# hilo-mpc/hilo-mpc

Hardware: AMD Instinct MI355X
Metric: MPC steps/sec (batched instances, whole node) at fixed (nx,nu,N) (higher is better)
Workload: dtype f64

## Files before the change

hilo_mpc_amd/csrc/hilo_nmpc_track.h:

```cpp
#pragma once
#include "hilo_ocp.h"

namespace hilo {

template <class M, bool BIG_ = false, bool SYM_ = true>
struct NmpcTrack {
  using Model = M;
  static constexpr bool SYM = SYM_ && ModelSym<M>::value && !model_has_ext<M>::value;
  static constexpr int NX = M::NX, NU = M::NU, NZ = NX + NU, NPAR = M::NP + M::NU, NSD = 0;
  static constexpr bool FIX_X0 = true;
  static constexpr bool BIG = BIG_;
  static constexpr int NC = 0, NXV = NX, NX0 = NX, NU0 = NU;
  static constexpr bool COOP = model_has_ext<M>::value;
  static constexpr bool QUAD_COST = true;
  static constexpr int O_WZ = 0, O_ZREF = O_WZ + NZ * NZ, O_WN = O_ZREF + NZ, O_XREFN = O_WN + NX * NX,
                       O_WDU = O_XREFN + NX, O_HASDU = O_WDU + NU * NU, O_SZ = O_HASDU + 1, O_SDU = O_SZ + NZ * NZ;
  static constexpr bool SYMTAB = O_SDU + NU * NU <= OCP_NCOST;
  static constexpr int O_END = SYMTAB ? O_SDU + NU * NU : O_SZ;
  static constexpr int NCOST = O_END;

  template <class T, class E>
  __device__ __forceinline__ static void dyn(const OcpConst& pc, const double* par, const double*, int, const T* x,
                                             const T* u, T* xn, const E& ext) {
    T xp[NX], up[NU > 0 ? NU : 1], xo[NX];
#pragma unroll
    for (int i = 0; i < NX; ++i) xp[i] = x[i] * pc.sz[i];
#pragma unroll
    for (int i = 0; i < NU; ++i) up[i] = u[i] * pc.sz[NX + i];
    model_step<M>(pc.order, pc.nsub, xp, up, par, pc.dt, xo, ext);
#pragma unroll
    for (int i = 0; i < NX; ++i) xn[i] = xo[i] * rcp_fast(pc.sz[i]);
  }

  static constexpr bool PLANT = !COOP;
  __device__ __forceinline__ static void plant(const OcpConst& pc, const double* par, const double* x, const double* u, double* xn) {
    if constexpr (PLANT) {
      double xv[NX], uv[NU > 0 ? NU : 1], pv[M::NP > 0 ? M::NP : 1], xo[NX];
#pragma unroll
      for (int i = 0; i < NX; ++i) xv[i] = x[i];
#pragma unroll
      for (int i = 0; i < NU; ++i) uv[i] = u[i];
#pragma unroll
      for (int i = 0; i < M::NP; ++i) pv[i] = par[i];
      model_step<M>(pc.order, pc.nsub, xv, uv, pv, pc.dt, xo);
#pragma unroll
      for (int i = 0; i < NX; ++i) xn[i] = xo[i];
    }
  }

  template <class T>
  __device__ __forceinline__ static T stage_cost(const OcpConst& pc, const double* par, const double*, int k,
                                                 const T* x, const T* u) {
    T z[NZ];
#pragma unroll
// ... 10 lines not shown
        for (int j = 0; j < NZ; ++j) w[a][j] = pc.cost[O_WZ + (i0 + a < NZ ? i0 + a : i0) * NZ + j];
      asm volatile("");
#pragma unroll
      for (int a = 0; a < 2; ++a) {
        if (i0 + a < NZ) {
          T s = T(0.0);
#pragma unroll
          for (int j = 0; j < NZ; ++j) s = s + w[a][j] * z[j];
          acc = acc + z[i0 + a] * s;
        }
      }
    }
    if (k == 0 && pc.cost[O_HASDU] != 0.0) {
      T d[NU > 0 ? NU : 1];
#pragma unroll
      for (int i = 0; i < NU; ++i) d[i] = u[i] - par[M::NP + i];
#pragma unroll
      for (int i = 0; i < NU; ++i) {
        T s = T(0.0);
#pragma unroll
        for (int j = 0; j < NU; ++j) s = s + pc.cost[O_WDU + i * NU + j] * d[j];
        acc = acc + d[i] * s;
      }
    }
    return acc;
  }

  __device__ __forceinline__ static double cost_grad(const OcpConst& pc, const double* par, const double*, int k, int i, const double* z) {
    double g = 0.0;
    {
      double wr[NZ], wc[NZ], zr[NZ];
#pragma unroll
      for (int j = 0; j < NZ; ++j) { wr[j] = pc.cost[O_WZ + i * NZ + j]; wc[j] = pc.cost[O_WZ + j * NZ + i]; zr[j] = pc.cost[O_ZREF + j]; }
      asm volatile("");
#pragma unroll
      for (int j = 0; j < NZ; ++j) g += (wr[j] + wc[j]) * (z[j] - zr[j]);
    }
    if (k == 0 && i >= NX && pc.cost[O_HASDU] != 0.0) {
#pragma unroll
      for (int j = 0; j < NU; ++j)
        g += (pc.cost[O_WDU + (i - NX) * NU + j] + pc.cost[O_WDU + j * NU + (i - NX)]) * (z[NX + j] - par[M::NP + j]);
    }
    return g;
  }
  __device__ __forceinline__ static double cost_hess(const OcpConst& pc, int k, int i, int j) {
    double h = pc.cost[O_WZ + i * NZ + j] + pc.cost[O_WZ + j * NZ + i];
// ... 88 lines not shown
```

hilo_mpc_amd/csrc/hilo_ocp.h:

```cpp
#pragma once
#include "hilo_colloc.h"
#include "hilo_common.h"
#include "hilo_models.h"

namespace hilo {

constexpr int OCP_MAXNX = 12, OCP_MAXNU = 8, OCP_MAXNZ = OCP_MAXNX + OCP_MAXNU;
constexpr int OCP_FILTER = 16;
constexpr int OCP_MAXNC = 16;
#ifndef HILO_OCP_TPB
#define HILO_OCP_TPB 64
#endif
#ifndef HILO_OCP_MINW
#define HILO_OCP_MINW 1
#endif
#ifdef HILO_OCP_INLINE_PHASES
#define OCP_PHASE __attribute__((always_inline))
#else
#define OCP_PHASE __attribute__((noinline))
#endif
constexpr int OCP_TPB = HILO_OCP_TPB;
constexpr int OCP_NCOST = 2 * OCP_MAXNZ * OCP_MAXNZ + 4 * OCP_MAXNZ + 64;

struct OcpConst {
// ... 156 lines not shown
template <class PB, class = void> struct pb_nh { static constexpr int value = 0; };
template <class PB> struct pb_nh<PB, void_tt<decltype(PB::NH)>> { static constexpr int value = PB::NH; };
template <class PB, class = void> struct pb_sym { static constexpr bool value = false; };
template <class PB> struct pb_sym<PB, void_tt<decltype(PB::SYM)>> { static constexpr bool value = PB::SYM; };
template <class PB, class = void> struct pb_sym_mhe { static constexpr bool value = false; };
template <class PB> struct pb_sym_mhe<PB, void_tt<decltype(PB::SYM_MHE)>> { static constexpr bool value = PB::SYM_MHE; };
template <class PB, class = void> struct pb_vec_n { static constexpr int value = 0; };
template <class PB> struct pb_vec_n<PB, void_tt<decltype(PB::VEC_N)>> { static constexpr int value = PB::VEC_N; };
template <class PB, class = void> struct pb_fused_con { static constexpr bool value = false; };
template <class PB> struct pb_fused_con<PB, void_tt<decltype(PB::FUSED_CON)>> { static constexpr bool value = PB::FUSED_CON; };
template <class PB, class = void> struct pb_prep { static constexpr int value = 0; };
template <class PB> struct pb_prep<PB, void_tt<decltype(PB::PREP)>> { static constexpr int value = PB::PREP; };
template <class PB, class = void> struct pb_vec_max { static constexpr int value = 3; };
template <class PB> struct pb_vec_max<PB, void_tt<decltype(PB::VEC_MAX)>> { static constexpr int value = PB::VEC_MAX; };
template <class PB, class = void> struct pb_cstage { static constexpr int value = 0; };
template <class PB> struct pb_cstage<PB, void_tt<decltype(PB::CSTAGE)>> { static constexpr int value = PB::CSTAGE; };
template <class PB, class = void> struct pb_xcw { static constexpr int value = 0; };
template <class PB> struct pb_xcw<PB, void_tt<decltype(PB::XCW)>> { static constexpr int value = PB::XCW; };
template <class PB, class = void> struct pb_lam_fix { static constexpr bool value = false; };
template <class PB> struct pb_lam_fix<PB, void_tt<decltype(PB::LAM_FIX)>> { static constexpr bool value = PB::LAM_FIX; };
template <class PB, class = void> struct pb_fused { static constexpr bool value = false; };
template <class PB> struct pb_fused<PB, void_tt<decltype(PB::FUSED)>> { static constexpr bool value = PB::FUSED; };

__host__ __device__ constexpr size_t ocp_iter_doubles(int NX, int NU, int NC, int N) {
  const size_t NZ = NX + NU, NDIR = NZ * (NZ + 1) / 2, S = (size_t)(N + 1) * NZ;
  return 9 * S + NX + 5 * (size_t)N * NX + (size_t)N * NX * (NZ + 1) + (size_t)N * NZ * (NZ + 1) + (size_t)(N + 1) * NDIR +
         (size_t)(N + 1) * NX * (NX + 1) + (size_t)N * NU * (NX + 1) + (size_t)N * NX * (NX + 1) + (size_t)N * NC * (14 + NZ) +
         (size_t)N * 4 * NX;
}
__host__ __device__ constexpr size_t ocp_fixed_doubles(int NX, int NU, int NCONST, int NPAR, int NSD, int NEXT, int N, int NPREP = 0) {
  const size_t NZ = NX + NU;
  return NCONST + NZ * NZ + NZ + (N + 1) + 2 * 16 + 16 + NPAR + (size_t)(N + 1) * (NSD > 0 ? NSD : 0) + 1 + NEXT +
         (NZ * (NZ + 1) / 2 + 2) / 2 + NPREP;
}

struct OcpExtra {
  const double* par2;
  int npar1;
  int gather_stride;
  double* v_copy;
  double* gather;
  double* lam_x;
  double* g;
  const double* lbx;
  const double* ubx;
  long long bx_stride;
  double* x_next;
};

#ifdef HILO_OCP_DPROF
__device__ long long g_dprof[32];
#define DTICK(i) { if (blockIdx.x == 0 && threadIdx.x == 0) { const long long tn_ = clock64(); g_dprof[i] += tn_ - dt_; dt_ = tn_; } }
#define DTICK0 long long dt_ = clock64();
#define DTICKR dt_ = clock64();
#else
#define DTICK(i)
// ... 8 lines not shown
  static constexpr int NX = PB::NX, NU = PB::NU, NZ = NX + NU, NDIR = NZ * (NZ + 1) / 2, NXDIR = NX * (NX + 1) / 2;
  static constexpr int NPAR = PB::NPAR > 0 ? PB::NPAR : 1, NSD = PB::NSD;
  static constexpr bool FIX_X0 = PB::FIX_X0;
  static constexpr int NH = pb_nh<PB>::value;
  static constexpr bool FUSED = pb_fused<PB>::value;
  static constexpr bool FUSED_CON = pb_fused_con<PB>::value;
  static constexpr int PREP = pb_prep<PB>::value;
  static constexpr int XCW = pb_xcw<PB>::value;
#ifndef HILO_OCP_PREPB
#define HILO_OCP_PREPB 3
#endif
  static constexpr int PREPB = XCW > 0 ? HILO_OCP_PREPB : 1;
  static constexpr int PREPL = PREP * PREPB > pb_cstage<PB>::value ? PREP * PREPB : pb_cstage<PB>::value;
  static constexpr bool SYM = pb_sym<PB>::value;
  static constexpr bool SYM_MHE = pb_sym_mhe<PB>::value;
  static constexpr bool COOP = PB::COOP;
  static constexpr int NEXT_SCR = COOP ? 12 * OCP_TPB : 0;
  static constexpr int NEXT = COOP ? NEXT_SCR + GP2_HDR + 3 * GP2_MAXN : 0;
  static constexpr int NC = PB::NC;
  static_assert(NC <= OCP_MAXNC, "too many constraint rows");
  static constexpr int NXV = PB::NXV, NX0 = PB::NX0, NU0 = PB::NU0;
  static_assert(!COOP || (OCP_TPB == 64 && NDIR <= 64), "cooperative models need one wave per instance");
  static constexpr bool MFMA_STAGE = OCP_TPB == 64 && NZ + 1 <= 16 && NX <= 16;
  static constexpr int NCONST = (int)((__builtin_offsetof(OcpConst, cost) + sizeof(double) * PB::NCOST + 7) / 8);
  static constexpr int ABP = NZ + 1, WP = NZ + 1, PP = NX + 1;

  static constexpr bool BIG = PB::BIG;
  using dp = cond_t<BIG, gbl_double*, lds_double*>;
  using cdp = cond_t<BIG, gbl_cdouble*, lds_cdouble*>;
  static constexpr int VEC_N = pb_vec_n<PB>::value;
  __host__ __device__ static constexpr size_t vec_doubles_level(int N, int level) {
    return (level >= 1 ? 7 * (size_t)(N + 1) * NZ : 0) + (level >= 2 ? 3 * (size_t)N * NX : 0) + (level >= 3 ? (size_t)(N + 1) * NZ : 0);
  }
  static constexpr size_t VEC_BUDGET = 40 * 1024 - 64;
  static constexpr bool vec_fits(int level) {
    return (ocp_fixed_doubles(NX, NU, NCONST, NPAR, NSD, NEXT, VEC_N, PREPL) + vec_doubles_level(VEC_N, level)) * sizeof(double) <= VEC_BUDGET;
  }
  static constexpr int VEC_FIT = !(BIG && VEC_N > 0) ? 0 : (vec_fits(3) ? 3 : (vec_fits(2) ? 2 : (vec_fits(1) ? 1 : 0)));
  static constexpr int VEC_LEVEL = VEC_FIT < pb_vec_max<PB>::value ? VEC_FIT : pb_vec_max<PB>::value;
  static constexpr bool VEC_LDS = VEC_LEVEL > 0;
  __host__ __device__ static constexpr size_t vec_doubles(int N) { return vec_doubles_level(N, VEC_LEVEL); }
  using vp = cond_t<BIG && VEC_LEVEL < 1, gbl_double*, lds_double*>;
  using cvp = cond_t<BIG && VEC_LEVEL < 1, gbl_cdouble*, lds_cdouble*>;
  using ep = cond_t<BIG && VEC_LEVEL < 2, gbl_double*, lds_double*>;
  using gp_t = cond_t<BIG && VEC_LEVEL < 3, gbl_double*, lds_double*>;
  struct Lds {
    const __attribute__((address_space(3))) OcpConst* pc;
    vp Z, Zt, D, zL, zU;
    vp lbA, ubA;
    ep lam, c, ct;
    gp_t grad;
    dp lamn, AB, W, Qd, P, Kg, sig, rbN, Acl;
    dp Xs;
    dp prep;
    dp xc;
    lds_double* prepl;
    lds_double* gpc;
    dp cs, cst, cnu, cnun, cvL, cvU, cdvL, cdvU, cds, cd, csig, crb, Jd;
    dp c0, cd0, cdt;
    lds_double *Mm, *mm, *fk, *filt, *red, *par, *sd, *ext;
    __attribute__((address_space(3))) int* dirs;
  };
  static_assert(OCP_FILTER == 16, "ocp_fixed_doubles assumes a filter of 16 entries");
  __host__ __device__ static constexpr size_t qd_doubles(int N) { return (SYM || SYM_MHE) ? (size_t)NXDIR : (size_t)(N + 1) * NDIR; }
  __host__ __device__ static constexpr size_t xs_doubles(int N) { return SYM ? (size_t)N * 4 * NX : (COOP ? (size_t)N * 24 : 0); }
  __host__ __device__ static constexpr size_t iter_doubles(int N) {
    return ocp_iter_doubles(NX, NU, NC, N) - (size_t)(N + 1) * NDIR - (size_t)N * 4 * NX + qd_doubles(N) + xs_doubles(N) +
           (size_t)N * PREP + (size_t)N * XCW;
  }
  __device__ static dp qd_term(const Lds l, int N) { return (SYM || SYM_MHE) ? l.Qd : l.Qd + (size_t)N * NDIR; }
  __host__ __device__ static constexpr size_t fixed_doubles(int N) {
    return ocp_fixed_doubles(NX, NU, NCONST, NPAR, NSD, NEXT, N, PREPL);
  }
  __host__ __device__ static constexpr size_t lds_doubles(int N) {
    return fixed_doubles(N) + (BIG ? (VEC_LDS ? vec_doubles(N) : 0) : iter_doubles(N));
  }
  __host__ __device__ static constexpr size_t ws_doubles(int N) { return BIG ? iter_doubles(N) - (VEC_LDS ? vec_doubles(N) : 0) : 0; }
  __device__ static int horizon_of(lds_double* base) {
    return reinterpret_cast<const __attribute__((address_space(3))) OcpConst*>(base)->N;
  }
  __device__ static Lds carve(lds_double* base, double* ws) { return carve(base, ws, horizon_of(base)); }
  __device__ static Lds carve(lds_double* base, double* ws, int N) {
    Lds l;
    const size_t S = (size_t)(N + 1) * NZ;
    lds_double* q = base;
    auto take = [&](size_t n) { lds_double* r = q; q += n; return r; };
    l.pc = reinterpret_cast<const __attribute__((address_space(3))) OcpConst*>(take(NCONST));
    l.Mm = take(NZ * NZ); l.mm = take(NZ);
    l.fk = take(N + 1); l.filt = take(2 * OCP_FILTER); l.red = take(16); l.par = take(NPAR);
    l.sd = take((size_t)(N + 1) * (NSD > 0 ? NSD : 0) + 1);
    l.ext = take(NEXT);
    l.dirs = reinterpret_cast<__attribute__((address_space(3))) int*>(take((NDIR + 2) / 2));
    l.prepl = take(PREPL);
    dp w;
    const size_t V = (size_t)N * NX;
    if constexpr (VEC_LEVEL >= 1) {
      l.Z = take(S); l.Zt = take(S); l.D = take(S); l.zL = take(S); l.zU = take(S); l.lbA = take(S); l.ubA = take(S);
    }
    if constexpr (VEC_LEVEL >= 2) { l.lam = take(V); l.c = take(V); l.ct = take(V); }
    if constexpr (VEC_LEVEL >= 3) l.grad = take(S);
    if constexpr (BIG) w = (gbl_double*)ws; else w = q;
    auto big = [&](size_t n) { dp r = w; w += n; return r; };
    if constexpr (VEC_LEVEL < 1) {
      l.Z = big(S); l.Zt = big(S); l.D = big(S); l.zL = big(S); l.zU = big(S); l.lbA = big(S); l.ubA = big(S);
    }
    if constexpr (VEC_LEVEL < 2) { l.lam = big(V); l.c = big(V); l.ct = big(V); }
    if constexpr (VEC_LEVEL < 3) l.grad = big(S);
    l.lamn = big((size_t)N * NX);
    l.AB = big((size_t)N * NX * ABP); l.W = big((size_t)N * NZ * WP); l.Qd = big(qd_doubles(N));
    l.P = big((size_t)(N + 1) * NX * PP);
// ... 62 lines not shown
      ii += go ? 1 : 0;
    }
    i = ii;
    j = ii + 1 + r;
  }
  __device__ static int dir_of(int i, int j, int n) { return n + i * (n - 1) - i * (i - 1) / 2 + (j - i - 1); }
  __device__ static bool pair_on(const OcpConst& pc, int d) {
    const int p = d - NZ;
    return p >= 256 || ((pc.pair_mask[p >> 6] >> (p & 63)) & 1ull) != 0ull;
  }
  __device__ static void build_dirs(const Lds l) {
    const OcpConst& pc = *(const OcpConst*)l.pc;
    if (threadIdx.x == 0) {
      int n = 0;
      for (int d = 0; d < NDIR; ++d)
        if (d < NZ || pair_on(pc, d)) l.dirs[1 + n++] = d;
      l.dirs[0] = n;
    }
    __syncthreads();
  }

  __device__ static const double* sd_of(const Lds l, int k) { return (const double*)(l.sd + (NSD > 0 ? k * NSD : 0)); }

  __device__ OCP_PHASE static FTheta eval_values_call(lds_double* lbase, double* ws, cvp Zp, ep cp, cdp sp, dp dstore, double extra) {
    lbase = uni(lbase); ws = uni(ws); Zp = uni(Zp); cp = uni(cp); sp = uni(sp); dstore = uni(dstore);
    const Lds l = carve(lbase, ws);
    const OcpConst& pc = *(const OcpConst*)l.pc;
    const int N = pc.N;
    double fpart = 0.0, tpart = 0.0;
    if constexpr (COOP) {
      const int lane = threadIdx.x;
      int gs = 64 / N;
      gs = gs < 1 ? 1 : gs;
      const int ng = 64 / gs, g = lane / gs, gl = lane - g * gs;
      const double* gp = (const double*)pc.ext;
      for (int r = 0; r * ng < N; ++r) {
        const int k = r * ng + g;
        const bool active = g < ng && k < N;
        const int kk = active ? k : N - 1;
        int nev = 0;
        const GpExt ext{gp, l.ext, gs, active ? gl : 0, active ? g * gs : lane, !active, (lds_cdouble*)(l.ext + NEXT_SCR),
                        pc.nsub == 1 ? l.gpc + kk * 24 : nullptr, &nev, false};
        double x[NX], u[NU > 0 ? NU : 1], xn[NX];
#pragma unroll
        for (int i = 0; i < NX; ++i) x[i] = Zp[kk * NZ + i];
#pragma unroll
        for (int i = 0; i < NU; ++i) u[i] = Zp[kk * NZ + NX + i];
        PB::dyn(pc, (const double*)l.par, sd_of(l, kk), kk, x, u, xn, ext);
        if (active && gl == 0) {
          fpart += PB::stage_cost(pc, (const double*)l.par, sd_of(l, k), k, x, u);
#pragma unroll
          for (int i = 0; i < NX; ++i) {
            const double ci = Zp[(k + 1) * NZ + i] - xn[i];
// ... 10 lines not shown
      }
    } else {
    if constexpr (XCW > 0) PB::template coll_pass<false>(pc, (const double*)l.par, (const double*)l.sd, Zp, l.lam, l.cnu, N, l.xc, l.prep, l.prepl,
                                                         uni((size_t)Zp != (size_t)l.Z));
#ifdef HILO_DBG_TWICE_VALS
    if constexpr (XCW > 0) PB::template coll_pass<false>(pc, (const double*)l.par, (const double*)l.sd, Zp, l.lam, l.cnu, N, l.xc, l.prep, l.prepl);
#endif
    OCP_FOR(k, (N) + 1) {
      double x[NX], u[NU > 0 ? NU : 1];
#pragma unroll
      for (int i = 0; i < NX; ++i) x[i] = Zp[k * NZ + i];
      if (k < N) {
        double xn[NX];
#pragma unroll
        for (int i = 0; i < NU; ++i) u[i] = Zp[k * NZ + NX + i];
        double dvf[NC > 0 ? NC : 1];
        if constexpr (XCW > 0) {
          fpart += PB::dyn_cost_xc(pc, (const double*)l.par, sd_of(l, k), k, x, u, xn, dvf, l.xc + (size_t)k * XCW);
        } else if constexpr (FUSED_CON) {
          static_assert(!FUSED_CON || FUSED, "fused rows need the fused cost");
          fpart += PB::dyn_cost_con(pc, (const double*)l.par, sd_of(l, k), k, x, u, xn, dvf, NoExt{});
        } else if constexpr (FUSED) {
          fpart += PB::dyn_cost(pc, (const double*)l.par, sd_of(l, k), k, x, u, xn, NoExt{});
        } else if constexpr (SYM) {
          using M = typename PB::Model;
          double xp[NX], up[NU > 0 ? NU : 1], X[4][NX], phi[NX];
#pragma unroll
          for (int i = 0; i < NX; ++i) xp[i] = x[i] * pc.sz[i];
#pragma unroll
          for (int i = 0; i < NU; ++i) up[i] = u[i] * pc.sz[NX + i];
          sym_points<M>(M::DISCRETE ? 1 : pc.order, pc.dt, xp, up, (const double*)l.par, X, phi);
          dp xs = l.Xs + (size_t)k * 4 * NX;
#pragma unroll
          for (int i = 0; i < 4; ++i)
#pragma unroll
            for (int q = 0; q < NX; ++q) xs[i * NX + q] = X[i][q];
#pragma unroll
          for (int i = 0; i < NX; ++i) xn[i] = phi[i] * rcp_fast(pc.sz[i]);
          fpart += PB::stage_cost(pc, (const double*)l.par, sd_of(l, k), k, x, u);
        } else {
          if constexpr (SYM_MHE) {
            FastD xf[NX], uf[NU > 0 ? NU : 1], xnf[NX];
#pragma unroll
            for (int i = 0; i < NX; ++i) xf[i] = FastD(x[i]);
#pragma unroll
            for (int i = 0; i < NU; ++i) uf[i] = FastD(u[i]);
            PB::dyn(pc, (const double*)l.par, sd_of(l, k), k, xf, uf, xnf, NoExt{});
#pragma unroll
            for (int i = 0; i < NX; ++i) xn[i] = xnf[i].v;
          } else {
            PB::dyn(pc, (const double*)l.par, sd_of(l, k), k, x, u, xn, NoExt{});
          }
          fpart += PB::stage_cost(pc, (const double*)l.par, sd_of(l, k), k, x, u);
        }
#pragma unroll
        for (int i = 0; i < NX; ++i) {
          const double ci = Zp[(k + 1) * NZ + i] - xn[i];
          cp[k * NX + i] = ci;
          tpart += fabs(ci);
        }
        if constexpr (NC > 0) {
          double dv[NC];
// ... 6 lines not shown
            if (row_on(pc, k, m)) {
              if (dstore) dstore[k * NC + m] = dv[m];
              if (sp) tpart += fabs(dv[m] - sp[k * NC + m]);
            }
          }
        }
      } else {
        fpart += PB::term_cost(pc, (const double*)l.par, sd_of(l, N), x);
      }
    }
    }
    if constexpr (OCP_TPB == 64) {
      double rv[3] = {fpart, tpart, extra};
      WaveReduceN<R_SUM, R_SUM, R_SUM>::run(rv);
      return FTheta{rv[0], rv[1], rv[2]};
    } else {
      const double fr = block_reduce<OpSum>(fpart, l.red);
      const double tr = block_reduce<OpSum>(tpart, l.red);
      return FTheta{fr, tr, block_reduce<OpSum>(extra, l.red)};
    }
  }

  __device__ __forceinline__ static FTheta eval_values(lds_double* lbase, double* ws, cvp Zp, ep cp, cdp sp = nullptr,
                                                      dp dstore = nullptr, double extra = 0.0) {
    const FTheta r = eval_values_call(lbase, ws, Zp, cp, sp, dstore, extra);
    return FTheta{uni(r.f), uni(r.theta), uni(r.x)};
  }

  template <bool TRIAL>
  __device__ __forceinline__ static double slots_log(const Lds l, cvp Zp, double alpha, int N) {
    constexpr int U = 2;
    const int SLT = (N + 1) * NZ;
    double part = 0.0;
    for (int base = 0; base < SLT; base += OCP_TPB * U) {
      double lbv[U], ubv[U], zv[U], dv[U];
      bool ok[U];
#pragma unroll
      for (int u = 0; u < U; ++u) {
        const int e0 = base + u * OCP_TPB + (int)threadIdx.x;
        ok[u] = e0 < SLT;
        const int e = ok[u] ? e0 : 0;
        lbv[u] = l.lbA[e]; ubv[u] = l.ubA[e]; zv[u] = Zp[e];
        dv[u] = TRIAL ? l.D[e] : 0.0;
      }
      double prod = 1.0;
      bool pos = true;
#pragma unroll
      for (int u = 0; u < U; ++u) {
        const double z = TRIAL ? zv[u] + alpha * dv[u] : zv[u];
        if constexpr (TRIAL) {
          if (ok[u]) l.Zt[base + u * OCP_TPB + (int)threadIdx.x] = z;
        }
        const bool hl = ok[u] && lbv[u] > -INFINITY, hu = ok[u] && ubv[u] < INFINITY;
        const double sl = hl ? z - lbv[u] : 1.0, su = hu ? ubv[u] - z : 1.0;
        prod *= sl * su;
        pos = pos && sl > 0.0 && su > 0.0;
      }
      const double r = -log(prod);
      part += pos ? r : __builtin_nan("");
    }
    return part;
  }
  __device__ static double barrier_logs(const Lds l, cvp Zp, cdp sp = nullptr) {
    const OcpConst& pc = *(const OcpConst*)l.pc;
    const int N = pc.N;
    double part = slots_log<false>(l, Zp, 0.0, N);
    if constexpr (NC > 0) {
      OCP_FOR(e, N * NC) {
        const int m = e % NC;
        if (!row_on(pc, e / NC, m)) continue;
        if (pc.dlb[m] > -INFINITY) part -= log(sp[e] - pc.dlb[m]);
        if (pc.dub[m] < INFINITY) part -= log(pc.dub[m] - sp[e]);
      }
    }
    return uni(block_reduce<OpSum>(part, l.red));
  }
  __device__ static double form_trial_part(const Lds l, double alpha) {
    const OcpConst& pc = *(const OcpConst*)l.pc;
    const int N = pc.N;
    double part = slots_log<true>(l, l.Z, alpha, N);
    if constexpr (NC > 0) {
      OCP_FOR(e, N * NC) {
        const int m = e % NC;
        const double sv = l.cs[e] + alpha * l.cds[e];
        l.cst[e] = sv;
        if (!row_on(pc, e / NC, m)) continue;
        if (pc.dlb[m] > -INFINITY) part -= log(sv - pc.dlb[m]);
        if (pc.dub[m] < INFINITY) part -= log(pc.dub[m] - sv);
      }
    }
    __syncthreads();
    return part;
  }

  __device__ __attribute__((always_inline)) static double eval_derivs_body(lds_double* lbase, double* ws, bool reuse = false) {
    const Lds l = carve(lbase, ws);
    const OcpConst& pc = *(const OcpConst*)l.pc;
    const int N = pc.N;
    const unsigned pinm = FIX_X0 ? (~pc.x0_free_mask) & ((1u << NX) - 1u) : 0u;
    constexpr int GPW = COOP ? 64 / NDIR : 1;
    const int nact = COOP ? NDIR : uni(l.dirs[0]);
    const int PASSES = (nact + OCP_TPB - 1) / OCP_TPB;
    const int ntask = COOP ? ((N + GPW - 1) / GPW) * 64 + NXDIR : (PREP > 0 ? N * PASSES * OCP_TPB + NXDIR : N * nact + NXDIR);
    const int tbase = ntask - NXDIR;
    if constexpr (XCW > 0) {
      PB::template coll_pass<true>(pc, (const double*)l.par, (const double*)l.sd, l.Z, l.lam, l.cnu, N, l.xc, l.prep, l.prepl);
#ifdef HILO_DBG_TWICE_COLL
      PB::template coll_pass<true>(pc, (const double*)l.par, (const double*)l.sd, l.Z, l.lam, l.cnu, N, l.xc, l.prep, l.prepl);
#endif
    } else if constexpr (PREP > 0) {
      OCP_FOR(k, N) {
        double x[NX], u[NU > 0 ? NU : 1];
#pragma unroll
        for (int i = 0; i < NX; ++i) x[i] = l.Z[k * NZ + i];
#pragma unroll
// ... 213 lines not shown
      OCP_FOR(e, N * NZ) {
        const int k = e / NZ, i = e - k * NZ;
        if (is_free(pc, k, i)) l.grad[e] = PB::cost_grad(pc, (const double*)l.par, sd_of(l, k), k, i, (const double*)(l.Z + k * NZ));
      }
      OCP_FOR(k, N) {
        double x[NX], u[NU > 0 ? NU : 1];
#pragma unroll
        for (int i = 0; i < NX; ++i) x[i] = l.Z[k * NZ + i];
#pragma unroll
        for (int i = 0; i < NU; ++i) u[i] = l.Z[k * NZ + NX + i];
        l.fk[k] = PB::stage_cost(pc, (const double*)l.par, sd_of(l, k), k, x, u);
      }
      __syncthreads();
    }
    double fpart = 0.0;
    OCP_FOR(k, (N) + 1) fpart += l.fk[k];
    OCP_FOR(a, NU) l.grad[N * NZ + NX + a] = 0.0;
    const double f = block_reduce<OpSum>(fpart, l.red);
    __syncthreads();
    return f;
  }


  template <class M>
  __device__ __forceinline__ static void sym_points(int order, double h, const double* x, const double* u, const double* par,
                                                    double (*X)[NX], double* phi) {
    constexpr bool DISC = M::DISCRETE;
    const double a10 = order >= 2 ? 0.5 : 0.0, a20 = order == 3 ? -1.0 : 0.0, a21 = order == 3 ? 2.0 : (order == 4 ? 0.5 : 0.0),
                 a32 = order == 4 ? 1.0 : 0.0;
    const double hb[4] = {DISC ? 1.0 : h * erk_b<0>(order), DISC ? 0.0 : h * erk_b<1>(order), DISC ? 0.0 : h * erk_b<2>(order),
                          DISC ? 0.0 : h * erk_b<3>(order)};
    FastD kk[4][NX], uf[NU > 0 ? NU : 1];
#pragma unroll
    for (int i = 0; i < NU; ++i) uf[i] = FastD(u[i]);
#pragma unroll
    for (int i = 0; i < 4; ++i) {
      FastD Xf[NX];
#pragma unroll
      for (int s = 0; s < NX; ++s) {
        double acc = x[s];
        if (i == 1) acc += (h * a10) * kk[0][s].v;
        if (i == 2) acc += (h * a20) * kk[0][s].v + (h * a21) * kk[1][s].v;
        if (i == 3) acc += (h * a32) * kk[2][s].v;
        X[i][s] = acc;
        Xf[s] = FastD(acc);
      }
      if (i < order) {
        M::ode(Xf, uf, par, h, kk[i]);
      } else {
#pragma unroll
// ... 33 lines not shown
    const double a10 = order >= 2 ? 0.5 : 0.0, a20 = order == 3 ? -1.0 : 0.0, a21 = order == 3 ? 2.0 : (order == 4 ? 0.5 : 0.0),
                 a32 = order == 4 ? 1.0 : 0.0;
    const double hb[4] = {DISC ? 1.0 : h * erk_b<0>(order), DISC ? 0.0 : h * erk_b<1>(order), DISC ? 0.0 : h * erk_b<2>(order),
                          DISC ? 0.0 : h * erk_b<3>(order)};
    const double* par = (const double*)l.par;
    DTICK0
    double fpart = 0.0;
    OCP_FOR(a, NU) l.grad[N * NZ + NX + a] = 0.0;
    DTICK(7)
    constexpr int IPP = OCP_TPB / LPI;
    static_assert(IPP >= 1, "SYM: more column groups than lanes");
    for (int kbase = 0; kbase < N; kbase += IPP) {
      const int li = (int)threadIdx.x / LPI;
      const bool act = li < IPP && kbase + li < N;
      const int k = act ? kbase + li : N - 1, g = act ? (int)threadIdx.x - li * LPI : 0, c0 = g * CPL;
      double zs[NZ], sz[NZ], isz[NX], x[NX], u[NU > 0 ? NU : 1], lamp[NX], X[4][NX], kb[4][NX];
#pragma unroll
      for (int i = 0; i < NZ; ++i) {
        zs[i] = l.Z[k * NZ + i];
        sz[i] = pc.sz[i];
      }
#pragma unroll
      for (int i = 0; i < NX; ++i) {
        isz[i] = rcp_fast(sz[i]);
        x[i] = zs[i] * sz[i];
        lamp[i] = l.lam[k * NX + i] * isz[i];
      }
#pragma unroll
      for (int i = 0; i < NU; ++i) u[i] = zs[NX + i] * sz[NX + i];
      DTICK(4)
      double ch[NZ][CPL];
      {
        double xN[NX];
#pragma unroll
        for (int i = 0; i < NX; ++i) xN[i] = l.Z[N * NZ + i];
        if constexpr (pb_symtab<PB>::value) {
          double gc[CPL];
          PB::template cost_cols<CPL>(pc, par, k, c0, zs, gc, ch);
          if (act) {
            if (g == 0 && !reuse) fpart += PB::stage_cost(pc, par, sd_of(l, k), k, zs, zs + NX);
            if (g == 0 && k == N - 1 && !reuse) fpart += PB::term_cost(pc, par, sd_of(l, N), xN);
#pragma unroll
            for (int c = 0; c < CPL; ++c) {
              const int col = c0 + c;
              if (col < NZ) l.grad[k * NZ + col] = is_free(pc, k, col) ? gc[c] : 0.0;
              if (col < NX && k == N - 1) l.grad[N * NZ + col] = PB::term_grad(pc, col, xN);
            }
// ... 182 lines not shown
    const OcpConst& pc = *(const OcpConst*)l.pc;
    const int N = pc.N, order = pc.order;
    const double h = pc.dt;
    const double a10 = order >= 2 ? 0.5 : 0.0, a20 = order == 3 ? -1.0 : 0.0, a21 = order == 3 ? 2.0 : (order == 4 ? 0.5 : 0.0),
                 a32 = order == 4 ? 1.0 : 0.0;
    const double hb[4] = {h * erk_b<0>(order), h * erk_b<1>(order), h * erk_b<2>(order), h * erk_b<3>(order)};
    const double* par = (const double*)l.par;
    double fpart = 0.0;
    OCP_FOR(d, NXDIR) qd_term(l, N)[d] = 0.0;
    OCP_FOR(a, NZ) l.grad[N * NZ + a] = 0.0;
    constexpr int IPP = OCP_TPB / LPI;
    for (int kbase = 0; kbase < N; kbase += IPP) {
      const int li = (int)threadIdx.x / LPI;
      const bool act = li < IPP && kbase + li < N;
      const int k = act ? kbase + li : N - 1, g = act ? (int)threadIdx.x - li * LPI : 0, c0 = g * CPL;
      const double* sd = sd_of(l, k);
      double xsv[NX], wv[NX], sz[NX], sw[NX], isz[NX], x[NX], ue[MU1], lamp[NX], X[4][NX], kb[4][NX];
#pragma unroll
      for (int i = 0; i < NX; ++i) {
        xsv[i] = l.Z[k * NZ + i];
        wv[i] = l.Z[k * NZ + NX + i];
        sz[i] = pc.sz[i];
        sw[i] = pc.sz[NX + i];
        isz[i] = rcp_fast(sz[i]);
        x[i] = xsv[i] * sz[i];
        lamp[i] = l.lam[k * NX + i] * isz[i];
      }
#pragma unroll
      for (int i = 0; i < MU; ++i) ue[i] = sd[i] * pc.cost[PB::O_SU + i];
      double chx[NX][CPL], chw[NX][CPL], gx[CPL], gw[CPL];
      {
        double Jy[NY * NX], Hy[NX * (NX + 1) / 2], kby[NY], r[NY], yv[NY], ws_[NX];
        double val = 0.0;
        if (k == 0) {
          double d[NX];
#pragma unroll
          for (int i = 0; i < NX; ++i) d[i] = x[i] - par[NP + i];
#pragma unroll
          for (int i = 0; i < NX; ++i)
#pragma unroll
            for (int j = 0; j < NX; ++j) val += d[i] * pc.cost[PB::O_WX + i * NX + j] * d[j];
#pragma unroll
          for (int c = 0; c < CPL; ++c) {
            const int col = c0 + c;
            double gacc = 0.0;
#pragma unroll
            for (int j = 0; j < NX; ++j) gacc += (pc.cost[PB::O_WX + col * NX + j] + pc.cost[PB::O_WX + j * NX + col]) * d[j];
// ... 547 lines not shown
      double s = y[a];
#pragma unroll
      for (int q = 0; q < a; ++q) s -= L[a * n + q] * y[q];
      y[a] = s * invd[a];
    }
#pragma unroll
    for (int a = n - 1; a >= 0; --a) {
      double s = y[a];
#pragma unroll
      for (int q = a + 1; q < n; ++q) s -= L[q * n + a] * y[q];
      y[a] = s * invd[a];
    }
  }

  static constexpr int KB_ = (NX + 3) / 4, RB_ = (NZ + 3) / 4;
#ifndef HILO_RIC_DUP
#define HILO_RIC_DUP 1
#endif
#ifndef HILO_RIC_TADD
#define HILO_RIC_TADD 1
#endif
#ifndef HILO_FWD_SGPR
#define HILO_FWD_SGPR 1
#endif
  static constexpr bool DUPU = HILO_RIC_DUP && OCP_TPB == 64 && NZ + 1 <= 16 && NX <= 16 && NU >= 1 && NU <= 2 && NH == 0 && NZ % 4 != 0 &&
                               RB_ + NU <= 4;
  static constexpr int RD_ = DUPU ? RB_ + NU : RB_;
  __device__ __forceinline__ static int stage_row(int r, int g) {
    if (DUPU && r >= RB_) return NX + (r - RB_);
    const int i = g + 4 * r;
    return (NZ % 4 == 0 || i < NZ) ? i : NZ - 1;
  }
  struct StageOps {
    double b1[KB_], bi[KB_][NU > 0 ? NU : 1];
    v4d M0;
  };
  struct PivotInv { double i0, i1, l; bool ok; };
#ifndef HILO_RCP_PIVOT_NEWTON
#define HILO_RCP_PIVOT_NEWTON 2
#endif
  __device__ __forceinline__ static double rcp_pivot(double x) {
    double r = __builtin_amdgcn_rcp(x);
#pragma unroll
    for (int q = 0; q < HILO_RCP_PIVOT_NEWTON; ++q) r = fma(fma(-x, r, 1.0), r, r);
    return r;
  }
// ... 665 lines not shown
        const bool pin = x0_pinned(pc, i) || x0_pinned(pc, j);
        l.Mm[e] = pin ? (i == j ? 1.0 : 0.0) : l.P[i * PP + j];
      }
      __syncthreads();
      double Lc[NX * NX], invd[NX], y[NX];
      const bool pd = small_chol<NX>(l.Mm, NX, Lc, invd);
      if (!pd) return false;
#pragma unroll
      for (int a = 0; a < NX; ++a) y[a] = x0_pinned(pc, a) ? 0.0 : l.P[a * PP + NX];
      small_solve<NX>(Lc, invd, y);
      __syncthreads();
      if (t == 0) {
#pragma unroll
        for (int a = 0; a < NX; ++a) l.D[a] = -y[a];
      }
    }
    DTICK(9)
    if constexpr (NU == 0) OCP_FOR(e, N * NX * PP) {
      const int row = e / PP, j = e - row * PP;
      l.Acl[e] = l.AB[(size_t)row * ABP + (j < NX ? j : NZ)];
    }
    __syncthreads();
#if HILO_FWD_SGPR
    if (t < 64) {
      constexpr int FU = 4;
      const int i = t < NX ? t : 0;
      double dxs[NX];
      {
        const double d0 = l.D[i];
#pragma unroll
        for (int j = 0; j < NX; ++j) dxs[j] = read_lane(d0, j);
      }
      double ca[FU][NX + 1], cb[FU][NX + 1];
      auto fetch = [&](double (&dst)[FU][NX + 1], int k0) __attribute__((always_inline)) {
#pragma unroll
        for (int q = 0; q < FU; ++q) {
          const int kq = k0 + q < N ? k0 + q : N - 1;
          cdp row = l.Acl + ((size_t)kq * NX + i) * PP;
#pragma unroll
          for (int j = 0; j <= NX; ++j) dst[q][j] = row[j];
        }
      };
      auto run = [&](const double (&c)[FU][NX + 1], int k0) __attribute__((always_inline)) {
        auto one = [&](int q, int k) __attribute__((always_inline)) {
          double s = c[q][NX], s2 = 0.0;
#pragma unroll
// ... 213 lines not shown
__device__ __forceinline__ void ocp_solve_body(lds_double* lds_raw, const OcpConst* __restrict__ pcg, int64_t batch,
                                               const double* __restrict__ x0, const double* __restrict__ par,
                                               int64_t par_stride, const double* __restrict__ sdata,
                                               int64_t sd_stride, const double* __restrict__ v0,
                                               int64_t v0_stride, int v0_prefix, int v_prefix, double* __restrict__ v_opt,
                                               double* __restrict__ f_opt, double* __restrict__ lam_g,
                                               double* __restrict__ first, int first_kind,
                                               int32_t* __restrict__ status, int32_t* __restrict__ iters,
                                               double* __restrict__ kkt, long long* __restrict__ prof,
                                               double* __restrict__ ws, const OcpExtra ex = OcpExtra(), int64_t b_in = -1,
                                               int64_t ws_slot = -1) {
  using S = Ocp<PB>;
  constexpr int NX = S::NX, NU = S::NU, NZ = S::NZ, NC = S::NC, NXV = S::NXV, NH = S::NH, NTAIL = NX - NXV - NH;
  const int t = threadIdx.x;
  const int64_t b = b_in >= 0 ? b_in : (int64_t)blockIdx.x;
  if (b >= batch) return;
  const int N = pcg->N;
  double* const wsb = ws ? ws + (ws_slot >= 0 ? ws_slot : b) * (int64_t)S::ws_doubles(N) : nullptr;
  typename S::Lds l = S::carve(lds_raw, wsb, N);
  {
    const double* src = reinterpret_cast<const double*>(pcg);
    lds_double* dst = lds_raw;
    OCP_FOR(i, S::NCONST) dst[i] = src[i];
  }
  {
    const int n1 = ex.par2 || ex.npar1 > 0 ? ex.npar1 : PB::NPAR;
    OCP_FOR(i, PB::NPAR) {
      double v = 0.0;
      if (i < n1) v = par[b * par_stride + i];
      else if (ex.par2) v = ex.par2[b * (int64_t)(PB::NPAR - n1) + (i - n1)];
      l.par[i] = v;
    }
  }
  if constexpr (PB::NSD > 0)
    OCP_FOR(i, (N + 1) * PB::NSD) l.sd[i] = sdata[b * sd_stride + i];
  if constexpr (S::COOP) {
    const double* gsrc = pcg->ext;
    const int nt = GP2_HDR + 3 * (int)gsrc[0];
    OCP_FOR(i, nt) l.ext[S::NEXT_SCR + i] = gsrc[i];
  }
  __syncthreads();
  const OcpConst& pc = *(const OcpConst*)l.pc;
  const int SL = (N + 1) * NZ;
  long long tprof[PH_COUNT] = {0, 0, 0, 0, 0, 0, 0, 0};
  long long tlast = prof ? clock64() : 0;
#define OCP_TICK(ph) if (prof) { const long long tn = clock64(); tprof[ph] += tn - tlast; tlast = tn; }
// ... 198 lines not shown
        l.cdvU[e] = du;
      }
    }
    DTICK(15)
    if constexpr (OCP_TPB == 64) {
      double rv[3] = {r_p, r_z, dphi};
      WaveReduceN<R_MAX, R_MAX, R_SUM>::run(rv);
      r_p = rv[0]; r_z = rv[1]; dphi = rv[2];
    } else {
      r_p = block_reduce<OpMax>(r_p, l.red);
      r_z = block_reduce<OpMax>(r_z, l.red);
      dphi = block_reduce<OpSum>(dphi, l.red);
    }
    const double a_p = uni(r_p > tau ? tau / r_p : 1.0), a_z = uni(r_z > tau ? tau / r_z : 1.0);
    if (!blog_ok) blog = S::barrier_logs(l, l.Z, l.cs);
    const double phi0 = uni(fval + mu * blog);
    DTICK(16)
    OCP_TICK(PH_STEP)
    double alpha = a_p;
    bool accepted = false, armijo = false;
    double blog_t = 0.0, f_acc = 0.0;
    for (int ls = 0; ls < 60; ++ls) {
      DTICKR
      const double blog_part = S::form_trial_part(l, alpha);
      DTICK(17)
      tprof[PH_NLS] += 1;
      const FTheta trial = S::eval_values(lds_raw, wsb, l.Zt, l.ct, l.cst, l.cdt, blog_part);
      blog_t = trial.x;
      DTICK(18)
      const double ft = trial.f, tht = trial.theta;
      const double pht = uni(ft + mu * blog_t);
      bool ok = isfinite(pht) && isfinite(tht) && tht <= theta_max;
      if (ok) {
        for (int q = 0; q < nfilt; ++q) {
          const double tf = l.filt[2 * q], pf = l.filt[2 * q + 1];
          if (tht >= tf && pht - 10 * 2.220446049250313e-16 * fabs(pf) >= pf) { ok = false; break; }
        }
      }
      bool sw = false;
      if (ok) {
        sw = th0 <= theta_min && dphi < 0.0 && S::switching(pc, alpha, -dphi, th0);
        const double rnd = 10 * 2.220446049250313e-16 * fabs(phi0);
        if (sw) ok = pht - phi0 - rnd <= pc.eta_phi * alpha * dphi;
        else ok = tht <= (1 - pc.gamma_theta) * th0 || pht - phi0 - rnd <= -pc.gamma_phi * th0;
      }
      DTICK(19)
      if (ok) { accepted = true; armijo = sw; f_acc = ft; break; }
      if (ls == 0 && tht >= th0) {
        OCP_FOR(e, N * NX) l.c0[e] = l.c[e];
        if constexpr (NC > 0)
// ... 6 lines not shown
            OCP_FOR(e, N * NC) {
              if (S::row_on(pc, e / NC, e % NC)) l.cd[e] = l.cs[e] + a_prev * (l.cd[e] - l.cs[e]) + (l.cdt[e] - l.cst[e]);
            }
          }
          __syncthreads();
          tprof[PH_NRIC] += 1;
          if (!uni(S::riccati(lds_raw, wsb, mu, delta))) break;
          double a = 1.0;
          OCP_FOR(e, SL) {
            const double d = l.D[e], lb = l.lbA[e], ub = l.ubA[e], z = l.Z[e];
            if (lb > -INFINITY && d < 0.0) a = fmin(a, -tau * (z - lb) / d);
            if (ub < INFINITY && d > 0.0) a = fmin(a, tau * (ub - z) / d);
          }
          if constexpr (NC > 0) {
            OCP_FOR(e, N * NC) {
              const int m = e % NC;
              if (!S::row_on(pc, e / NC, m)) continue;
              const double d = l.cds[e];
              if (pc.dlb[m] > -INFINITY && d < 0.0) a = fmin(a, -tau * (l.cs[e] - pc.dlb[m]) / d);
              if (pc.dub[m] < INFINITY && d > 0.0) a = fmin(a, tau * (pc.dub[m] - l.cs[e]) / d);
            }
          }
          const double a_s = block_reduce<OpMin>(a, l.red);
          const double blog_part2 = S::form_trial_part(l, a_s);
          tprof[PH_NLS] += 1;
          const FTheta t2 = S::eval_values(lds_raw, wsb, l.Zt, l.ct, l.cst, l.cdt, blog_part2);
          blog_t = t2.x;
          const double ths = t2.theta;
          const double phs = uni(t2.f + mu * blog_t);
          bool oks = isfinite(phs) && isfinite(ths) && ths <= theta_max;
          if (oks) {
            for (int q = 0; q < nfilt; ++q) {
              const double tf = l.filt[2 * q], pf = l.filt[2 * q + 1];
              if (ths >= tf && phs - 10 * 2.220446049250313e-16 * fabs(pf) >= pf) { oks = false; break; }
            }
          }
          if (oks) {
            const bool sw2 = th0 <= theta_min && dphi < 0.0 && S::switching(pc, alpha, -dphi, th0);
            const double rnd = 10 * 2.220446049250313e-16 * fabs(phi0);
            if (sw2) oks = phs - phi0 - rnd <= pc.eta_phi * alpha * dphi;
            else oks = ths <= (1 - pc.gamma_theta) * th0 || phs - phi0 - rnd <= -pc.gamma_phi * th0;
            if (oks) { soc_ok = true; soc_sw = sw2; f_acc = t2.f; break; }
          }
          if (!(ths <= 0.99 * th_old)) break;
          th_old = ths;
          a_prev = a_s;
        }
        if (soc_ok) {
          OCP_FOR(e, N * NX) {
// ... 274 lines not shown
```

Baseline: 6.516 million.

## Restructure SYM trial evaluation, cache inverse scales, add lane-local forward sweep

```diff
diff --git a/hilo_mpc_amd/csrc/hilo_nmpc_track.h b/hilo_mpc_amd/csrc/hilo_nmpc_track.h
--- a/hilo_mpc_amd/csrc/hilo_nmpc_track.h
+++ b/hilo_mpc_amd/csrc/hilo_nmpc_track.h
@@ -28,8 +28,9 @@
 #pragma unroll
     for (int i = 0; i < NU; ++i) up[i] = u[i] * pc.sz[NX + i];
     model_step<M>(pc.order, pc.nsub, xp, up, par, pc.dt, xo, ext);
-#pragma unroll
-    for (int i = 0; i < NX; ++i) xn[i] = xo[i] * rcp_fast(pc.sz[i]);
+    const double* isz = ocp_isz<NCOST>(pc);
+#pragma unroll
+    for (int i = 0; i < NX; ++i) xn[i] = xo[i] * isz[i];
   }
 
   static constexpr bool PLANT = !COOP;
@@ -86,6 +87,70 @@
         for (int j = 0; j < NU; ++j) s = s + pc.cost[O_WDU + i * NU + j] * d[j];
         acc = acc + d[i] * s;
       }
+    }
+    return acc;
+  }
+
+  struct CostOps {
+    double wz[NZ][NZ], zr[NZ], wn[NX][NX], xr[NX], wdu[NU > 0 ? NU : 1][NU > 0 ? NU : 1], hasdu;
+  };
+  __device__ __forceinline__ static void cost_ops(const OcpConst& pc, CostOps& o) {
+#pragma unroll
+    for (int i = 0; i < NZ; ++i)
+#pragma unroll
+      for (int j = 0; j < NZ; ++j) o.wz[i][j] = pc.cost[O_WZ + i * NZ + j];
+#pragma unroll
+    for (int i = 0; i < NZ; ++i) o.zr[i] = pc.cost[O_ZREF + i];
+#pragma unroll
+    for (int i = 0; i < NX; ++i)
+#pragma unroll
+      for (int j = 0; j < NX; ++j) o.wn[i][j] = pc.cost[O_WN + i * NX + j];
+#pragma unroll
+    for (int i = 0; i < NX; ++i) o.xr[i] = pc.cost[O_XREFN + i];
+#pragma unroll
+    for (int i = 0; i < NU; ++i)
+#pragma unroll
+      for (int j = 0; j < NU; ++j) o.wdu[i][j] = pc.cost[O_WDU + i * NU + j];
+    o.hasdu = pc.cost[O_HASDU];
+  }
+  __device__ __forceinline__ static double stage_cost_ops(const CostOps& o, const double* uold, int k, const double* x, const double* u) {
+    double z[NZ];
+#pragma unroll
+    for (int i = 0; i < NX; ++i) z[i] = x[i] - o.zr[i];
+#pragma unroll
+    for (int i = 0; i < NU; ++i) z[NX + i] = u[i] - o.zr[NX + i];
+    double acc = 0.0;
+#pragma unroll
+    for (int i = 0; i < NZ; ++i) {
+      double s = 0.0;
+#pragma unroll
+      for (int j = 0; j < NZ; ++j) s = s + o.wz[i][j] * z[j];
+      acc = acc + z[i] * s;
+    }
+    double accd = acc;
+    double d[NU > 0 ? NU : 1];
+#pragma unroll
+    for (int i = 0; i < NU; ++i) d[i] = u[i] - uold[i];
+#pragma unroll
+    for (int i = 0; i < NU; ++i) {
+      double s = 0.0;
+#pragma unroll
+      for (int j = 0; j < NU; ++j) s = s + o.wdu[i][j] * d[j];
+      accd = accd + d[i] * s;
+    }
+    return (k == 0 && o.hasdu != 0.0) ? accd : acc;
+  }
+  __device__ __forceinline__ static double term_cost_ops(const CostOps& o, const double* x) {
+    double z[NX];
+#pragma unroll
+    for (int i = 0; i < NX; ++i) z[i] = x[i] - o.xr[i];
+    double acc = 0.0;
+#pragma unroll
+    for (int i = 0; i < NX; ++i) {
+      double s = 0.0;
+#pragma unroll
+      for (int j = 0; j < NX; ++j) s = s + o.wn[i][j] * z[j];
+      acc = acc + z[i] * s;
     }
     return acc;
   }
diff --git a/hilo_mpc_amd/csrc/hilo_ocp.h b/hilo_mpc_amd/csrc/hilo_ocp.h
--- a/hilo_mpc_amd/csrc/hilo_ocp.h
+++ b/hilo_mpc_amd/csrc/hilo_ocp.h
@@ -202,6 +202,10 @@
 template <class PB, class = void> struct pb_fused { static constexpr bool value = false; };
 template <class PB> struct pb_fused<PB, void_tt<decltype(PB::FUSED)>> { static constexpr bool value = PB::FUSED; };
 
+__host__ __device__ constexpr int ocp_nconst(int ncost) { return (int)((__builtin_offsetof(OcpConst, cost) + sizeof(double) * ncost + 7) / 8); }
+template <int NCOST>
+__device__ __forceinline__ const double* ocp_isz(const OcpConst& pc) { return reinterpret_cast<const double*>(&pc) + ocp_nconst(NCOST); }
+
 __host__ __device__ constexpr size_t ocp_iter_doubles(int NX, int NU, int NC, int N) {
   const size_t NZ = NX + NU, NDIR = NZ * (NZ + 1) / 2, S = (size_t)(N + 1) * NZ;
   return 9 * S + NX + 5 * (size_t)N * NX + (size_t)N * NX * (NZ + 1) + (size_t)N * NZ * (NZ + 1) + (size_t)(N + 1) * NDIR +
@@ -211,7 +215,7 @@
 __host__ __device__ constexpr size_t ocp_fixed_doubles(int NX, int NU, int NCONST, int NPAR, int NSD, int NEXT, int N, int NPREP = 0) {
   const size_t NZ = NX + NU;
   return NCONST + NZ * NZ + NZ + (N + 1) + 2 * 16 + 16 + NPAR + (size_t)(N + 1) * (NSD > 0 ? NSD : 0) + 1 + NEXT +
-         (NZ * (NZ + 1) / 2 + 2) / 2 + NPREP;
+         (NZ * (NZ + 1) / 2 + 2) / 2 + NPREP + NZ;
 }
 
 struct OcpExtra {
@@ -266,7 +270,7 @@
   static constexpr int NXV = PB::NXV, NX0 = PB::NX0, NU0 = PB::NU0;
   static_assert(!COOP || (OCP_TPB == 64 && NDIR <= 64), "cooperative models need one wave per instance");
   static constexpr bool MFMA_STAGE = OCP_TPB == 64 && NZ + 1 <= 16 && NX <= 16;
-  static constexpr int NCONST = (int)((__builtin_offsetof(OcpConst, cost) + sizeof(double) * PB::NCOST + 7) / 8);
+  static constexpr int NCONST = ocp_nconst(PB::NCOST);
   static constexpr int ABP = NZ + 1, WP = NZ + 1, PP = NX + 1;
 
   static constexpr bool BIG = PB::BIG;
@@ -303,6 +307,7 @@
     dp cs, cst, cnu, cnun, cvL, cvU, cdvL, cdvU, cds, cd, csig, crb, Jd;
     dp c0, cd0, cdt;
     lds_double *Mm, *mm, *fk, *filt, *red, *par, *sd, *ext;
+    lds_double* isz;
     __attribute__((address_space(3))) int* dirs;
   };
   static_assert(OCP_FILTER == 16, "ocp_fixed_doubles assumes a filter of 16 entries");
@@ -330,6 +335,7 @@
     lds_double* q = base;
     auto take = [&](size_t n) { lds_double* r = q; q += n; return r; };
     l.pc = reinterpret_cast<const __attribute__((address_space(3))) OcpConst*>(take(NCONST));
+    l.isz = take(NZ);
     l.Mm = take(NZ * NZ); l.mm = take(NZ);
     l.fk = take(N + 1); l.filt = take(2 * OCP_FILTER); l.red = take(16); l.par = take(NPAR);
     l.sd = take((size_t)(N + 1) * (NSD > 0 ? NSD : 0) + 1);
@@ -438,13 +444,87 @@
 
   __device__ static const double* sd_of(const Lds l, int k) { return (const double*)(l.sd + (NSD > 0 ? k * NSD : 0)); }
 
-  __device__ OCP_PHASE static FTheta eval_values_call(lds_double* lbase, double* ws, cvp Zp, ep cp, cdp sp, dp dstore, double extra) {
+  struct SymUni {
+    int order;
+    double h, sz[NZ], isz[NX], par[NPAR];
+  };
+  template <int ORD, bool LOG>
+  __device__ __forceinline__ static void eval_values_sym_trip(const Lds l, const OcpConst& pc, int N, cvp Zp, ep cp, int k_base,
+                                                              const SymUni& un, double& fpart, double& tpart, double& extra, double lp) {
+    using M = typename PB::Model;
+    static_assert(NC == 0 && XCW == 0 && !COOP, "SYM: plain tracking policies");
+    const int k = k_base + (int)threadIdx.x;
+    const bool stage = k < N, last = k == N;
+    const int kx = k < N ? k : N, kn = k < N ? k + 1 : N;
+    double x[NX], u[NU > 0 ? NU : 1], xnx[NX];
+#pragma unroll
+    for (int i = 0; i < NX; ++i) x[i] = Zp[kx * NZ + i];
+#pragma unroll
+    for (int i = 0; i < NU; ++i) u[i] = Zp[kx * NZ + NX + i];
+#pragma unroll
+    for (int i = 0; i < NX; ++i) xnx[i] = Zp[kn * NZ + i];
+    double cost;
+    {
+      typename PB::CostOps co;
+      PB::cost_ops(pc, co);
+      asm volatile("");
+      const double sc = PB::stage_cost_ops(co, un.par + M::NP, k, x, u), tc = PB::term_cost_ops(co, x);
+      cost = stage ? sc : (last ? tc : 0.0);
+      asm volatile("" : "+v"(cost));
+    }
+    fpart += cost;
+    double xp[NX], up[NU > 0 ? NU : 1], X[4][NX], phi[NX], ci[NX];
+#pragma unroll
+    for (int i = 0; i < NX; ++i) xp[i] = x[i] * un.sz[i];
+#pragma unroll
+    for (int i = 0; i < NU; ++i) up[i] = u[i] * un.sz[NX + i];
+    sym_points<M, ORD>(un.order, un.h, xp, up, un.par, X, phi);
+#pragma unroll
+    for (int i = 0; i < NX; ++i) {
+      ci[i] = xnx[i] - phi[i] * un.isz[i];
+      tpart += stage ? fabs(ci[i]) : 0.0;
+    }
+    if constexpr (LOG) extra += -log(lp);
+    if (stage) {
+      dp xs = l.Xs + (size_t)k * 4 * NX;
+#pragma unroll
+      for (int i = 0; i < 4; ++i)
+#pragma unroll
+        for (int q = 0; q < NX; ++q) xs[i * NX + q] = X[i][q];
+#pragma unroll
+      for (int i = 0; i < NX; ++i) cp[k * NX + i] = ci[i];
+    }
+  }
+
+  __device__ OCP_PHASE static FTheta eval_values_call(lds_double* lbase, double* ws, cvp Zp, ep cp, cdp sp, dp dstore, double extra,
+                                                      double lprod) {
     lbase = uni(lbase); ws = uni(ws); Zp = uni(Zp); cp = uni(cp); sp = uni(sp); dstore = uni(dstore);
     const Lds l = carve(lbase, ws);
     const OcpConst& pc = *(const OcpConst*)l.pc;
     const int N = pc.N;
     double fpart = 0.0, tpart = 0.0;
-    if constexpr (COOP) {
+    if constexpr (SYM) {
+      using M = typename PB::Model;
+      SymUni un;
+      un.order = uni(M::DISCRETE ? 1 : pc.order);
+      un.h = uni(pc.dt);
+#pragma unroll
+      for (int i = 0; i < NZ; ++i) un.sz[i] = pc.sz[i];
+#pragma unroll
+      for (int i = 0; i < NX; ++i) un.isz[i] = l.isz[i];
+#pragma unroll
+      for (int i = 0; i < NPAR; ++i) un.par[i] = l.par[i];
+#pragma unroll
+      for (int i = 0; i < NZ; ++i) un.sz[i] = uni(un.sz[i]);
+#pragma unroll
+      for (int i = 0; i < NX; ++i) un.isz[i] = uni(un.isz[i]);
+#pragma unroll
+      for (int i = 0; i < NPAR; ++i) un.par[i] = uni(un.par[i]);
+      if (un.order == 4) eval_values_sym_trip<4, LOG_IN_EVAL>(l, pc, N, Zp, cp, 0, un, fpart, tpart, extra, lprod);
+      else eval_values_sym_trip<0, LOG_IN_EVAL>(l, pc, N, Zp, cp, 0, un, fpart, tpart, extra, lprod);
+      for (int k_base = OCP_TPB; k_base < N + 1; k_base += OCP_TPB)
+        eval_values_sym_trip<0, false>(l, pc, N, Zp, cp, k_base, un, fpart, tpart, extra, 1.0);
+    } else if constexpr (COOP) {
       const int lane = threadIdx.x;
       int gs = 64 / N;
       gs = gs < 1 ? 1 : gs;
@@ -501,22 +581,6 @@
           fpart += PB::dyn_cost_con(pc, (const double*)l.par, sd_of(l, k), k, x, u, xn, dvf, NoExt{});
         } else if constexpr (FUSED) {
           fpart += PB::dyn_cost(pc, (const double*)l.par, sd_of(l, k), k, x, u, xn, NoExt{});
-        } else if constexpr (SYM) {
-          using M = typename PB::Model;
-          double xp[NX], up[NU > 0 ? NU : 1], X[4][NX], phi[NX];
-#pragma unroll
-          for (int i = 0; i < NX; ++i) xp[i] = x[i] * pc.sz[i];
-#pragma unroll
-          for (int i = 0; i < NU; ++i) up[i] = u[i] * pc.sz[NX + i];
-          sym_points<M>(M::DISCRETE ? 1 : pc.order, pc.dt, xp, up, (const double*)l.par, X, phi);
-          dp xs = l.Xs + (size_t)k * 4 * NX;
-#pragma unroll
-          for (int i = 0; i < 4; ++i)
-#pragma unroll
-            for (int q = 0; q < NX; ++q) xs[i * NX + q] = X[i][q];
-#pragma unroll
-          for (int i = 0; i < NX; ++i) xn[i] = phi[i] * rcp_fast(pc.sz[i]);
-          fpart += PB::stage_cost(pc, (const double*)l.par, sd_of(l, k), k, x, u);
         } else {
           if constexpr (SYM_MHE) {
             FastD xf[NX], uf[NU > 0 ? NU : 1], xnf[NX];
@@ -569,13 +633,13 @@
   }
 
   __device__ __forceinline__ static FTheta eval_values(lds_double* lbase, double* ws, cvp Zp, ep cp, cdp sp = nullptr,
-                                                      dp dstore = nullptr, double extra = 0.0) {
-    const FTheta r = eval_values_call(lbase, ws, Zp, cp, sp, dstore, extra);
+                                                      dp dstore = nullptr, double extra = 0.0, double lprod = 1.0) {
+    const FTheta r = eval_values_call(lbase, ws, Zp, cp, sp, dstore, extra, lprod);
     return FTheta{uni(r.f), uni(r.theta), uni(r.x)};
   }
 
-  template <bool TRIAL>
-  __device__ __forceinline__ static double slots_log(const Lds l, cvp Zp, double alpha, int N) {
+  template <bool TRIAL, bool DEFER = false>
+  __device__ __forceinline__ static double slots_log(const Lds l, cvp Zp, double alpha, int N, double* lprod = nullptr) {
     constexpr int U = 2;
     const int SLT = (N + 1) * NZ;
     double part = 0.0;
@@ -603,8 +667,12 @@
         prod *= sl * su;
         pos = pos && sl > 0.0 && su > 0.0;
       }
-      const double r = -log(prod);
-      part += pos ? r : __builtin_nan("");
+      if (DEFER && base + OCP_TPB * U >= SLT) {
+        *lprod = pos ? prod : __builtin_nan("");
+      } else {
+        const double r = -log(prod);
+        part += pos ? r : __builtin_nan("");
+      }
     }
     return part;
   }
@@ -622,10 +690,16 @@
     }
     return uni(block_reduce<OpSum>(part, l.red));
   }
-  __device__ static double form_trial_part(const Lds l, double alpha) {
+#ifndef HILO_LOG_IN_EVAL
+#define HILO_LOG_IN_EVAL 1
+#endif
+  static constexpr bool LOG_IN_EVAL = HILO_LOG_IN_EVAL && SYM;
+  struct TrialPart { double part, prod; };
+  __device__ static TrialPart form_trial_part(const Lds l, double alpha) {
     const OcpConst& pc = *(const OcpConst*)l.pc;
     const int N = pc.N;
-    double part = slots_log<true>(l, l.Z, alpha, N);
+    double prod = 1.0;
+    double part = slots_log<true, LOG_IN_EVAL>(l, l.Z, alpha, N, &prod);
     if constexpr (NC > 0) {
       OCP_FOR(e, N * NC) {
         const int m = e % NC;
@@ -637,7 +711,7 @@
       }
     }
     __syncthreads();
-    return part;
+    return TrialPart{part, prod};
   }
 
   __device__ __attribute__((always_inline)) static double eval_derivs_body(lds_double* lbase, double* ws, bool reuse = false) {
@@ -897,10 +971,11 @@
   }
 
 
-  template <class M>
+  template <class M, int ORD = 0>
   __device__ __forceinline__ static void sym_points(int order, double h, const double* x, const double* u, const double* par,
                                                     double (*X)[NX], double* phi) {
     constexpr bool DISC = M::DISCRETE;
+    if constexpr (ORD > 0) order = ORD;
     const double a10 = order >= 2 ? 0.5 : 0.0, a20 = order == 3 ? -1.0 : 0.0, a21 = order == 3 ? 2.0 : (order == 4 ? 0.5 : 0.0),
                  a32 = order == 4 ? 1.0 : 0.0;
     const double hb[4] = {DISC ? 1.0 : h * erk_b<0>(order), DISC ? 0.0 : h * erk_b<1>(order), DISC ? 0.0 : h * erk_b<2>(order),
@@ -980,7 +1055,7 @@
       }
 #pragma unroll
       for (int i = 0; i < NX; ++i) {
-        isz[i] = rcp_fast(sz[i]);
+        isz[i] = l.isz[i];
         x[i] = zs[i] * sz[i];
         lamp[i] = l.lam[k * NX + i] * isz[i];
       }
@@ -1209,7 +1284,7 @@
         wv[i] = l.Z[k * NZ + NX + i];
         sz[i] = pc.sz[i];
         sw[i] = pc.sz[NX + i];
-        isz[i] = rcp_fast(sz[i]);
+        isz[i] = l.isz[i];
         x[i] = xsv[i] * sz[i];
         lamp[i] = l.lam[k * NX + i] * isz[i];
       }
@@ -1803,6 +1878,9 @@
 #endif
 #ifndef HILO_FWD_SGPR
 #define HILO_FWD_SGPR 1
+#endif
+#ifndef HILO_FWD_LANES
+#define HILO_FWD_LANES 1
 #endif
   static constexpr bool DUPU = HILO_RIC_DUP && OCP_TPB == 64 && NZ + 1 <= 16 && NX <= 16 && NU >= 1 && NU <= 2 && NH == 0 && NZ % 4 != 0 &&
                                RB_ + NU <= 4;
@@ -2514,6 +2592,61 @@
     }
     __syncthreads();
 #if HILO_FWD_SGPR
+    if constexpr (HILO_FWD_LANES && NX <= 4) {
+      if (t < 64) {
+        constexpr int FU = 1;
+        double dxs[NX];
+#pragma unroll
+        for (int j = 0; j < NX; ++j) dxs[j] = l.D[j];
+        double ca[FU][NX][NX + 1], cb[FU][NX][NX + 1];
+        auto fetch = [&](double (&dst)[FU][NX][NX + 1], int k0) __attribute__((always_inline)) {
+#pragma unroll
+          for (int q = 0; q < FU; ++q) {
+            const int kq = k0 + q < N ? k0 + q : N - 1;
+            cdp blk = l.Acl + (size_t)kq * NX * PP;
+#pragma unroll
+            for (int r = 0; r < NX; ++r)
+#pragma unroll
+              for (int j = 0; j <= NX; ++j) dst[q][r][j] = blk[r * PP + j];
+          }
+        };
+        auto run = [&](const double (&c)[FU][NX][NX + 1], int k0) __attribute__((always_inline)) {
+          auto one = [&](int q, int k) __attribute__((always_inline)) {
+            double sn[NX];
+#pragma unroll
+            for (int r = 0; r < NX; ++r) {
+              double s = c[q][r][NX], s2 = 0.0;
+#pragma unroll
+              for (int j = 0; j < NX; ++j) {
+                if (j & 1) s2 = fma(c[q][r][j], dxs[j], s2);
+                else s = fma(c[q][r][j], dxs[j], s);
+              }
+              sn[r] = s + s2;
+            }
+#pragma unroll
+            for (int r = 0; r < NX; ++r) {
+              l.D[(k + 1) * NZ + r] = sn[r];
+              dxs[r] = sn[r];
+            }
+          };
+          if (k0 + FU <= N) {
+#pragma unroll
+            for (int q = 0; q < FU; ++q) one(q, k0 + q);
+          } else {
+#pragma unroll
+            for (int q = 0; q < FU; ++q)
+              if (k0 + q < N) one(q, k0 + q);
+          }
+        };
+        fetch(ca, 0);
+        for (int k0 = 0; k0 < N; k0 += 2 * FU) {
+          fetch(cb, k0 + FU);
+          run(ca, k0);
+          fetch(ca, k0 + 2 * FU);
+          run(cb, k0 + FU);
+        }
+      }
+    } else
     if (t < 64) {
       constexpr int FU = 4;
       const int i = t < NX ? t : 0;
@@ -2773,6 +2906,7 @@
     const double* src = reinterpret_cast<const double*>(pcg);
     lds_double* dst = lds_raw;
     OCP_FOR(i, S::NCONST) dst[i] = src[i];
+    OCP_FOR(i, NZ) l.isz[i] = rcp_fast(pcg->sz[i]);
   }
   {
     const int n1 = ex.par2 || ex.npar1 > 0 ? ex.npar1 : PB::NPAR;
@@ -3017,10 +3151,10 @@
     double blog_t = 0.0, f_acc = 0.0;
     for (int ls = 0; ls < 60; ++ls) {
       DTICKR
-      const double blog_part = S::form_trial_part(l, alpha);
+      const typename S::TrialPart blog_part = S::form_trial_part(l, alpha);
       DTICK(17)
       tprof[PH_NLS] += 1;
-      const FTheta trial = S::eval_values(lds_raw, wsb, l.Zt, l.ct, l.cst, l.cdt, blog_part);
+      const FTheta trial = S::eval_values(lds_raw, wsb, l.Zt, l.ct, l.cst, l.cdt, blog_part.part, blog_part.prod);
       blog_t = trial.x;
       DTICK(18)
       const double ft = trial.f, tht = trial.theta;
@@ -3073,9 +3207,9 @@
             }
           }
           const double a_s = block_reduce<OpMin>(a, l.red);
-          const double blog_part2 = S::form_trial_part(l, a_s);
+          const typename S::TrialPart blog_part2 = S::form_trial_part(l, a_s);
           tprof[PH_NLS] += 1;
-          const FTheta t2 = S::eval_values(lds_raw, wsb, l.Zt, l.ct, l.cst, l.cdt, blog_part2);
+          const FTheta t2 = S::eval_values(lds_raw, wsb, l.Zt, l.ct, l.cst, l.cdt, blog_part2.part, blog_part2.prod);
           blog_t = t2.x;
           const double ths = t2.theta;
           const double phs = uni(t2.f + mu * blog_t);
```

Result: slower. 6.127 million (-6.0%).
